# zfwangDP/X2-GNN

Hardware: AMD Instinct MI355X
Metric: molecules/sec (fwd+bwd) on QM9 U0, batch=128, 1/2/4/8 MI355X (higher is better)
Workload: dtype fp32; 1 GPU; xgnn_poly U0 train step (config.json: L=4, D=128, H=16, sbf 7x6), S160, fwd+loss+bwd+allreduce+clip+Adam+EMA; per_gpu_batch=128, global_batch=128, line_nodes_per_gpu=21058, triplets_per_gpu=194060, parallelism=dp1, hip_graph=True

## Files before the change

### x2-gnn_amd/csrc/attention_center.hip

```cpp
#include <math.h>

#include <type_traits>

#include "common.hpp"
#include "../../include/x2g_staged.h"

namespace x2g {
namespace {

constexpr int kCD = 128;
constexpr float kCEps = 1e-16f;
typedef float cf4 __attribute__((ext_vector_type(4)));

__device__ __forceinline__ cf4 ld4(const float* p) { return *reinterpret_cast<const cf4*>(p); }
__device__ __forceinline__ void st4(float* p, cf4 v) { *reinterpret_cast<cf4*>(p) = v; }

template <int LPH>
__device__ __forceinline__ float head_sum(float v) {
  return group_sum<LPH>(v);
}

template <int LPH>
__device__ __forceinline__ float qk_logit(cf4 qv, cf4 kr, float sqrt_c) {
  float dot = __fmul_rn(qv[0], kr[0]);
  dot = __fmaf_rn(qv[1], kr[1], dot);
  dot = __fmaf_rn(qv[2], kr[2], dot);
  dot = __fmaf_rn(qv[3], kr[3], dot);
  return __fdiv_rn(head_sum<LPH>(dot), sqrt_c);
}

__device__ __forceinline__ float half_sum(float v, int half) {
  v = half32_sum_hi(v);
  const float lo = lane_bcast(v, 31), hi = lane_bcast(v, 63);
  return half ? hi : lo;
}

constexpr int kFactBatch = 4;
constexpr int kSfL = 7;
constexpr int kSfR = 6;
constexpr int kSfK = kSfL * kSfR;

constexpr int kMaxMembers = 32;

struct UnitRows {
  int* LN;
  int* RI;
  int* ER;
  int* MA;
  int* MI;
  int* NRS;
};

__host__ __device__ constexpr size_t unit_rows_lds(int rows) {
  return ((static_cast<size_t>(3) * rows + 2 * kMaxMembers + 4) * 4 + 15) / 16 * 16;
}

__device__ __forceinline__ UnitRows unit_rows_carve(int* p, int max_rows) {
  UnitRows u;
  u.NRS = p;
  u.MA = p + 4;
  u.MI = u.MA + kMaxMembers;
  u.LN = u.MI + kMaxMembers;
  u.RI = u.LN + max_rows;
  u.ER = u.RI + max_rows;
  return u;
}

__device__ __forceinline__ void unit_rows_build(const UnitRows& u, const int32_t* __restrict__ order,
                                                const int32_t* __restrict__ packs, int64_t unit,
                                                const int32_t* __restrict__ rowptr,
                                                const int32_t* __restrict__ src_row,
                                                const int4* __restrict__ info, int max_rows) {
  if (threadIdx.x >= 64) return;
  const int lane = threadIdx.x;
  int64_t m0 = unit, m1 = unit + 1;
  if (packs) {
    m0 = packs[unit];
    m1 = packs[unit + 1];
  }
  const int M = static_cast<int>(m1 - m0);
  int b = 0, r0 = 0, n = 0, er = 0;
  if (info) {
    if (lane < M) {
      const int4 v = info[m0 + lane];
      b = v.x;
      r0 = v.y;
      n = v.z;
      er = src_row ? v.w : 0;
    }
  } else {
    if (lane < M) {
      b = order ? order[m0 + lane] : static_cast<int>(m0 + lane);
      r0 = rowptr[b];
      n = rowptr[b + 1] - r0;
    }
    er = (src_row && n > 0) ? src_row[r0] : 0;
  }
  int inc = n;
#pragma unroll
  for (int o = 1; o < 64; o <<= 1) {
    const int v = __shfl_up(inc, o);
    if (lane >= o) inc += v;
  }
  const int base = inc - n;
  const int total = __shfl(inc, 63);
  if (total > max_rows) {
    if (lane == 63) {
      u.NRS[0] = 0;
      u.NRS[1] = 0;
    }
    return;
  }
  if (lane < M) {
    u.MA[lane] = b;
    u.MI[lane] = base | n << 16;
    for (int r = 0; r < n; ++r) {
      u.LN[base + r] = r0 + r;
      u.RI[base + r] = base | n << 16;
      u.ER[base + r] = er;
    }
  }
  if (lane == 63) {
    u.NRS[0] = inc;
    u.NRS[1] = M;
  }
}

struct FwdCenterArgs {
  const float *q, *k, *v, *skip, *edge;
  const int32_t* src_row;
  const float* sp;
  int64_t t_base;
  const int32_t *atom_rowptr, *edge_rev, *rev_trip;
  const int32_t* order;
  int64_t atom0, n_atoms;
  int H;
  float sqrt_c;
  float *out, *alpha, *smax, *sden;
  float2* row_stats;
};

template <int LPH, int WAVES, int B, bool EDGE>
__global__ void __launch_bounds__(64 * WAVES) attn_fwd_center_kernel(const FwdCenterArgs a) {
  extern __shared__ cf4 lds[];
  const int64_t b = a.order ? static_cast<int64_t>(a.order[a.atom0 + blockIdx.x]) : a.atom0 + blockIdx.x;
  const int r0 = uniform(a.atom_rowptr[b]);
  const int n = uniform(a.atom_rowptr[b + 1]) - r0;
  if (n <= 0) return;
  cf4* ke = lds;
  cf4* ve = lds + n * 32;
  const int tid = threadIdx.x;
  const int l32 = tid & 31, half = (tid >> 5) & 1, wave = tid >> 6;
  const int owner = 2 * wave + half;
  const int head = l32 / LPH;
  const bool leader = (l32 % LPH) == 0;
  const int c0 = 4 * l32;
  int i = owner;
  int d = 0, tb = 0;
// ... 424 lines not shown
          if constexpr (PREFETCH) load(j0 + B, yn, tn);
          cf4 sv[B];
          float lg[B];
          float mb = -INFINITY;
#pragma unroll
          for (int uu = 0; uu < B; ++uu) {
            const int j = j0 + uu;
            const bool ok = j < n && j != i;
            const int jr = (j < t1 ? j : t1 - 1) - t0;
            float yl[kSfL];
            yl[0] = dpp_mov<0x150>(yv[uu]);
            yl[1] = dpp_mov<0x151>(yv[uu]);
            yl[2] = dpp_mov<0x152>(yv[uu]);
            yl[3] = dpp_mov<0x153>(yv[uu]);
            yl[4] = dpp_mov<0x154>(yv[uu]);
            yl[5] = dpp_mov<0x155>(yv[uu]);
            yl[6] = dpp_mov<0x156>(yv[uu]);
            cf4 s4 = bias4;
            if constexpr (DROP && RMAX > 2 && B > 2) s4 = ld4(a.bias + c0);
#pragma unroll
            for (int l = 0; l < kSfL; ++l) s4 += yl[l] * P[(jr * kSfL + l) * 32 + l32];
            sv[uu] = s4;
            if constexpr (STORE) {
              if (a.sp && ok) st4(a.sp + static_cast<int64_t>(tt[uu]) * kCD + c0, s4);
            }
            const cf4 kr = KE[jr * 32 + l32];
            const float logit = qk_logit<LPH>(qv, kr, a.sqrt_c);
            lg[uu] = ok ? logit : -INFINITY;
            mb = fmaxf(mb, lg[uu]);
            if constexpr (STORE) {
              if (a.alpha && ok && leader) a.alpha[static_cast<int64_t>(tt[uu]) * a.H + head] = logit;
            }
          }
          const float m_new = fmaxf(m[r], mb);
          const float corr = m_new == -INFINITY ? 1.f : expf(m[r] - m_new);
          den[r] *= corr;
          acc[r] *= corr;
#pragma unroll
          for (int uu = 0; uu < B; ++uu) {
            const int j = j0 + uu;
            const float p = lg[uu] == -INFINITY ? 0.f : expf(lg[uu] - m_new);
            const cf4 vr = VE[((j < t1 ? j : t1 - 1) - t0) * 32 + l32];
            den[r] += p;
            if constexpr (DROP)
              acc[r] += (p * (drop_keep(dkey, tt[uu], head, a.H) ? dkey.scale : 0.f)) * (vr * sv[uu]);
            else
              acc[r] += p * (vr * sv[uu]);
          }
          m[r] = m_new;
          if constexpr (PREFETCH) {
#pragma unroll
            for (int uu = 0; uu < B; ++uu) {
              yv[uu] = yn[uu];
              tt[uu] = tn[uu];
            }
          } else {
            load(j0 + B, yv, tt);
          }
        }
      }
    }
  }
#pragma unroll
  for (int r = 0; r < RMAX; ++r) {
    if (owner + NO * r >= n) continue;
    const int dd = DDs[owner + NO * r];
    const int64_t drow = static_cast<int64_t>(dd) * kCD + c0;
    const float inv = 1.0f / (den[r] + kCEps);
    const cf4 o = acc[r] * inv + ld4(a.skip + drow);
    st4(a.out + drow, o);
    if (a.row_stats) {
      const float mu = half_sum(o[0] + o[1] + o[2] + o[3], half) / static_cast<float>(kCD);
      const cf4 dv = o - mu;
      const float q2 = half_sum(dv[0] * dv[0] + dv[1] * dv[1] + dv[2] * dv[2] + dv[3] * dv[3], half);
      if (l32 == 0) a.row_stats[dd] = make_float2(mu, q2);
    }
    if (leader) {
      a.smax[static_cast<int64_t>(dd) * a.H + head] = m[r];
      a.sden[static_cast<int64_t>(dd) * a.H + head] = den[r];
    }
  }
}

constexpr size_t fwd_sf_tiled_lds() {
  return static_cast<size_t>(kTileRows) * ((2 + kSfL) * kCD + kSfK) * 4 + 2 * X2G_CENTER_MAX_DEGREE * 4;
}

template <int LPH, bool DROP>
int fwd_sf_tiled_launch(const FwdSfArgs& a, bool edge, int max_degree, hipStream_t st) {
  constexpr int W = 8, B = 4;
  const size_t lds = fwd_sf_tiled_lds();
  const unsigned grid = static_cast<unsigned>(a.n_atoms);
  auto go = [&](auto kern) -> int {
    const hipError_t e = hipFuncSetAttribute(reinterpret_cast<const void*>(kern),
                                             hipFuncAttributeMaxDynamicSharedMemorySize, static_cast<int>(lds));
    if (e != hipSuccess) return static_cast<int>(e);
    kern<<<grid, 64 * W, lds, st>>>(a);
    return last_launch_status();
  };
  constexpr int NO = 2 * W;
  const bool store = a.alpha || a.sp || a.pp;
  auto pick = [&](auto rmax) -> int {
    constexpr int R = decltype(rmax)::value;
    if constexpr (DROP) {
      static_assert(R <= 4, "no RMAX 8 dropout instance");
      constexpr int BN = LPH == 1 && R > 2 ? 2 : B;
      return edge ? go(attn_fwd_center_sf_tiled_kernel<LPH, W, B, true, R, true, true>)
                  : go(attn_fwd_center_sf_tiled_kernel<LPH, W, BN, false, R, true, true>);
    } else {
      if (store)
        return edge ? go(attn_fwd_center_sf_tiled_kernel<LPH, W, B, true, R, true, false>)
                    : go(attn_fwd_center_sf_tiled_kernel<LPH, W, B, false, R, true, false>);
      return edge ? go(attn_fwd_center_sf_tiled_kernel<LPH, W, B, true, R, false, false>)
                  : go(attn_fwd_center_sf_tiled_kernel<LPH, W, B, false, R, false, false>);
    }
  };
  if (max_degree <= 2 * NO) return pick(std::integral_constant<int, 2>{});
  if (max_degree <= 4 * NO) return pick(std::integral_constant<int, 4>{});
  if constexpr (DROP)
    return X2G_EUNSUPPORTED;
  else
    return pick(std::integral_constant<int, 8>{});
}

template <int LPH>
int fwd_center_launch(const FwdCenterArgs& a, bool edge, int max_degree, hipStream_t st) {
  constexpr int W = 4, B = 8;
  const size_t lds = static_cast<size_t>(2) * max_degree * kCD * sizeof(float);
  const unsigned grid = static_cast<unsigned>(a.n_atoms);
  auto go = [&](auto kern) -> int {
    if (lds > 64 * 1024) {
      const hipError_t e = hipFuncSetAttribute(reinterpret_cast<const void*>(kern),
                                               hipFuncAttributeMaxDynamicSharedMemorySize, static_cast<int>(lds));
      if (e != hipSuccess) return static_cast<int>(e);
    }
    kern<<<grid, 64 * W, lds, st>>>(a);
    return last_launch_status();
  };
  return edge ? go(attn_fwd_center_kernel<LPH, W, B, true>) : go(attn_fwd_center_kernel<LPH, W, B, false>);
}

struct BwdCenterArgs {
  const float *q, *k, *v, *edge;
  const int32_t* src_row;
  const float *sp, *alpha, *smax, *sden, *dout, *y;
  const float *pp, *bias;
  const int32_t *atom_rowptr, *edge_rev, *rev_trip;
  const int32_t* order;
  int64_t n_atoms, T;
  int H;
  float inv_sqrt_c;
  float sqrt_c;
  float *dq, *dk, *dv, *gfold, *d_edge, *gw;
  const int64_t* drop_key;
  uint32_t drop_salt, drop_thr;
  float drop_scale;
};

template <int H>
__host__ __device__ constexpr size_t bwd_center_lds(int n) {
  return static_cast<size_t>(n) * 4 * kCD * 4
         + static_cast<size_t>(n) * H * 4 * 3
         + static_cast<size_t>(n) * 4 * 2;
}

template <int LPH, int WAVES, int B, bool EDGE, bool FACT, bool DROP>
__global__ void __launch_bounds__(64 * WAVES, 4) attn_bwd_center_kernel(const BwdCenterArgs a) {
  static_assert(FACT || !DROP, "the dropout instances are the P-row ones");
  constexpr int H = 32 / LPH;
  extern __shared__ cf4 lds[];
  const int64_t b = a.order ? static_cast<int64_t>(a.order[blockIdx.x]) : static_cast<int64_t>(blockIdx.x);
  const int r0 = uniform(a.atom_rowptr[b]);
  const int n = uniform(a.atom_rowptr[b + 1]) - r0;
  const int tid = threadIdx.x;
  const int l32 = tid & 31, half = (tid >> 5) & 1, wave = tid >> 6;
  const int owner = 2 * wave + half;
  constexpr int NO = 2 * WAVES;
  const int head = l32 / LPH;
  const bool leader = (l32 % LPH) == 0;
  const int c0 = 4 * l32;
  DropKey dkey{};
  if constexpr (DROP) dkey = drop_key(a.drop_key, a.drop_salt, a.drop_thr, a.drop_scale);
  if (n <= 0) {
    if (a.d_edge && tid < 32) st4(a.d_edge + b * kCD + c0, cf4{0.f, 0.f, 0.f, 0.f});
    return;
  }
  cf4* KE = lds;
  cf4* GO = KE + n * 32;
  cf4* QI = GO + n * 32;
  cf4* DE = QI + n * 32;
  float* MX = reinterpret_cast<float*>(DE + n * 32);
  float* IV = MX + n * H;
  float* RHO = IV + n * H;
  int* TB = reinterpret_cast<int*>(RHO + n * H);
  int* DI = TB + n;
  const int64_t e_row = EDGE ? static_cast<int64_t>(uniform(a.src_row[r0])) * kCD : 0;
  for (int idx = tid; idx < n; idx += 64 * WAVES) {
    TB[idx] = a.rev_trip[r0 + idx];
    DI[idx] = a.edge_rev[r0 + idx];
  }
  __syncthreads();
  constexpr int NT = 64 * WAVES;
  if (n * 32 <= 2 * NT && n * H <= NT) {
    cf4 kk[2], gg[2], qq[2];
    const int c = tid & 31;
    const cf4 e4 = EDGE ? ld4(a.edge + e_row + 4 * c) : cf4{0.f, 0.f, 0.f, 0.f};
#pragma unroll
    for (int u = 0; u < 2; ++u) {
      int j = (tid + u * NT) >> 5;
      j = j < n ? j : n - 1;
      const int64_t d = DI[j];
      kk[u] = ld4(a.k + static_cast<int64_t>(r0 + j) * kCD + 4 * c);
      gg[u] = ld4(a.dout + d * kCD + 4 * c);
      qq[u] = ld4(a.q + d * kCD + 4 * c);
    }
    const int sidx = tid < n * H ? tid : 0;
    const int si = sidx / H, sh = sidx - si * H;
    const int64_t sd = DI[si];
    const float mx = a.smax[sd * H + sh], dn = a.sden[sd * H + sh];
#pragma unroll
    for (int u = 0; u < 2; ++u) {
      const int idx = tid + u * NT;
      if (idx < n * 32) {
        KE[idx] = kk[u] + e4;
        GO[idx] = gg[u];
        QI[idx] = qq[u];
      }
    }
    if (tid < n * H) {
      MX[tid] = mx;
      IV[tid] = 1.0f / (dn + kCEps);
    }
  } else {
    for (int idx = tid; idx < n * 32; idx += NT) {
      const int j = idx >> 5, c = idx & 31;
      const int64_t d = DI[j];
      const cf4 e4 = EDGE ? ld4(a.edge + e_row + 4 * c) : cf4{0.f, 0.f, 0.f, 0.f};
      KE[idx] = ld4(a.k + static_cast<int64_t>(r0 + j) * kCD + 4 * c) + e4;
      GO[idx] = ld4(a.dout + d * kCD + 4 * c);
      QI[idx] = ld4(a.q + d * kCD + 4 * c);
    }
    for (int idx = tid; idx < n * H; idx += NT) {
      const int i = idx / H, h = idx - i * H;
      const int64_t d = DI[i];
      MX[idx] = a.smax[d * H + h];
      IV[idx] = 1.0f / (a.sden[d * H + h] + kCEps);
    }
  }
  __syncthreads();
  const int nt = n - 1;
  auto rsrc = [](const void* p, int64_t bytes) {
    return __builtin_amdgcn_make_buffer_rsrc(const_cast<void*>(p), static_cast<short>(0),
                                             static_cast<int>(bytes < 0x7fffffff ? bytes : 0x7fffffff), 0x00020000);
  };
  const __amdgpu_buffer_rsrc_t sp_r = rsrc(a.sp, a.T * kCD * 4);
  const __amdgpu_buffer_rsrc_t al_r = rsrc(a.alpha, a.T * H * 4);
  const __amdgpu_buffer_rsrc_t y_r = rsrc(a.y, a.T * 8 * 4);
  const __amdgpu_buffer_rsrc_t ag_r = rsrc(a.gw, a.T * H * 8);
  auto ldf = [](__amdgpu_buffer_rsrc_t r, int off) {
    return __builtin_bit_cast(float, __builtin_amdgcn_raw_buffer_load_b32(r, off, 0, 0));
  };
  auto ldag = [&](int t) {
    return __builtin_bit_cast(float2, __builtin_amdgcn_raw_buffer_load_b64(ag_r, (t * H + head) * 8, 0, 0));
  };
  auto trip = [&](int i, int j) {
    int pos = j - (j > i ? 1 : 0);
    pos = pos < nt ? pos : nt - 1;
    return TB[i] + pos;
  };
  for (int j = owner; j < n; j += NO) {
    const int64_t srow = static_cast<int64_t>(r0 + j) * kCD + c0;
    cf4 ue = ld4(a.v + srow);
    if (EDGE) ue += ld4(a.edge + e_row + c0);
    cf4 dv = {0.f, 0.f, 0.f, 0.f};
    cf4 pj[FACT ? kSfL : 1], bias4 = {0.f, 0.f, 0.f, 0.f};
    if constexpr (FACT) {
#pragma unroll
      for (int l = 0; l < kSfL; ++l) pj[l] = ld4(a.pp + (static_cast<int64_t>(r0 + j) * kSfL + l) * kCD + c0);
      bias4 = ld4(a.bias + c0);
    }
    auto batch = [&](int i0, auto bb) {
      constexpr int BB = decltype(bb)::value;
      cf4 sv[FACT ? 1 : BB];
      float yv[FACT ? BB : 1];
      float al[BB];
      int tt[BB];
#pragma unroll
      for (int u = 0; u < BB; ++u) {
        const int i = i0 + u < n ? i0 + u : n - 1;
        tt[u] = trip(i, j);
        if constexpr (FACT)
          yv[u] = ldf(y_r, (tt[u] * 8 + (l32 & 7)) * 4);
        else
          sv[u] = __builtin_bit_cast(cf4, __builtin_amdgcn_raw_buffer_load_b128(sp_r, tt[u] * (kCD * 4) + c0 * 4, 0, 0));
        al[u] = ldf(al_r, (tt[u] * H + head) * 4);
      }
#pragma unroll
      for (int u = 0; u < BB; ++u) {
        const int i = i0 + u < n ? i0 + u : n - 1;
        const bool ok = i0 + u < n && i != j;
        cf4 st;
        if constexpr (FACT) {
          float yl[kSfL];
          yl[0] = dpp_mov<0x150>(yv[u]);
          yl[1] = dpp_mov<0x151>(yv[u]);
          yl[2] = dpp_mov<0x152>(yv[u]);
          yl[3] = dpp_mov<0x153>(yv[u]);
          yl[4] = dpp_mov<0x154>(yv[u]);
          yl[5] = dpp_mov<0x155>(yv[u]);
          yl[6] = dpp_mov<0x156>(yv[u]);
          st = bias4;
#pragma unroll
          for (int l = 0; l < kSfL; ++l) st += yl[l] * pj[l];
        } else {
          st = sv[u];
        }
        const float at = ok ? expf(al[u] - MX[i * H + head]) * IV[i * H + head] : 0.f;
        const cf4 go = GO[i * 32 + l32];
        const cf4 gu = go * ue;
        float gp = gu[0] * st[0];
        gp = fmaf(gu[1], st[1], gp);
        gp = fmaf(gu[2], st[2], gp);
        gp = fmaf(gu[3], st[3], gp);
        const float g = head_sum<LPH>(gp);
        if (ok && leader) *reinterpret_cast<float2*>(a.gw + (static_cast<int64_t>(tt[u]) * H + head) * 2) = make_float2(g, at);
        dv += at * (go * st);
      }
    };
    if constexpr (FACT) {
      constexpr int BB = kFactBatch;
      if (nt > 0) {
        const cf4 kj = KE[j * 32 + l32];
        float yv[BB];
        int tt[BB];
        auto load = [&](int i0, float (&y_)[BB], int (&t_)[BB]) {
#pragma unroll
          for (int u = 0; u < BB; ++u) {
            const int i = i0 + u < n ? i0 + u : n - 1;
            t_[u] = trip(i, j);
            y_[u] = ldf(y_r, (t_[u] * 8 + (l32 & 7)) * 4);
          }
        };
        load(0, yv, tt);
        for (int i0 = 0; i0 < n; i0 += BB) {
          float yn[BB];
          int tn[BB];
          load(i0 + BB, yn, tn);
#pragma unroll
          for (int u = 0; u < BB; ++u) {
            const int i = i0 + u < n ? i0 + u : n - 1;
            const bool ok = i0 + u < n && i != j;
            float yl[kSfL];
            yl[0] = dpp_mov<0x150>(yv[u]);
            yl[1] = dpp_mov<0x151>(yv[u]);
            yl[2] = dpp_mov<0x152>(yv[u]);
            yl[3] = dpp_mov<0x153>(yv[u]);
            yl[4] = dpp_mov<0x154>(yv[u]);
            yl[5] = dpp_mov<0x155>(yv[u]);
            yl[6] = dpp_mov<0x156>(yv[u]);
            cf4 st = bias4;
#pragma unroll
            for (int l = 0; l < kSfL; ++l) st += yl[l] * pj[l];
            const float logit = qk_logit<LPH>(QI[i * 32 + l32], kj, a.sqrt_c);
            const float at = ok ? expf(logit - MX[i * H + head]) * IV[i * H + head] : 0.f;
            const cf4 go = GO[i * 32 + l32];
            const cf4 gu = go * ue;
            float gp = gu[0] * st[0];
            gp = fmaf(gu[1], st[1], gp);
            gp = fmaf(gu[2], st[2], gp);
            gp = fmaf(gu[3], st[3], gp);
            const float g = head_sum<LPH>(gp);
            if constexpr (DROP) {
              const float rk = drop_keep(dkey, tt[u], head, H) ? dkey.scale : 0.f;
              __builtin_amdgcn_raw_buffer_store_b64(__builtin_bit_cast(__attribute__((ext_vector_type(2))) unsigned,
                                                                       make_float2(g * rk, rk != 0.f ? at : -at)),
                                                    ag_r, (ok && leader) ? (tt[u] * H + head) * 8 : static_cast<int>(0x80000000u),
                                                    0, 0);
              dv += (at * rk) * (go * st);
            } else {
              __builtin_amdgcn_raw_buffer_store_b64(__builtin_bit_cast(__attribute__((ext_vector_type(2))) unsigned,
                                                                       make_float2(g, at)),
                                                    ag_r, (ok && leader) ? (tt[u] * H + head) * 8 : static_cast<int>(0x80000000u),
                                                    0, 0);
              dv += at * (go * st);
            }
          }
#pragma unroll
          for (int u = 0; u < BB; ++u) {
            yv[u] = yn[u];
            tt[u] = tn[u];
          }
        }
      }
    } else if (nt > 0) {
      int i0 = 0;
      for (; n - i0 > B / 2; i0 += B) batch(i0, std::integral_constant<int, B>{});
      if (i0 < n) batch(i0, std::integral_constant<int, B / 2>{});
    }
    st4(a.dv + srow, dv);
    DE[j * 32 + l32] = dv;
  }
  __threadfence_block();
  __syncthreads();
  for (int i = owner; i < n; i += NO) {
    float rho = 0.f;
    for (int p0 = 0; p0 < nt; p0 += 8) {
      float at[8], g[8];
#pragma unroll
      for (int u = 0; u < 8; ++u) {
        const float2 ag = ldag(TB[i] + (p0 + u < nt ? p0 + u : nt - 1));
        g[u] = ag.x;
        at[u] = ag.y;
      }
#pragma unroll
      for (int u = 0; u < 8; ++u)
        if (p0 + u < nt) {
          if constexpr (DROP)
            rho = fmaf(fabsf(at[u]), g[u], rho);
          else
            rho = fmaf(at[u], g[u], rho);
        }
    }
    if (leader) RHO[i * H + head] = rho;
  }
  __syncthreads();
  for (int o = owner; o < n; o += NO) {
    const int64_t srow = static_cast<int64_t>(r0 + o) * kCD + c0;
    cf4 ue = ld4(a.v + srow);
    if (EDGE) ue += ld4(a.edge + e_row + c0);
    cf4 dk = {0.f, 0.f, 0.f, 0.f}, dq = {0.f, 0.f, 0.f, 0.f};
    cf4 G[8];
#pragma unroll
    for (int l = 0; l < 8; ++l) G[l] = cf4{0.f, 0.f, 0.f, 0.f};
    const float rho_o = RHO[o * H + head];
    auto batch = [&](int x0, auto bb) {
      constexpr int BB = decltype(bb)::value;
      float ats[BB], gs[BB], yv[BB], atd[BB], gd[BB];
#pragma unroll
      for (int u = 0; u < BB; ++u) {
        const int x = x0 + u < n ? x0 + u : n - 1;
        const int ts = trip(x, o), td = trip(o, x);
        const float2 ags = ldag(ts), agd = ldag(td);
        gs[u] = ags.x;
        ats[u] = ags.y;
        yv[u] = ldf(y_r, (ts * 8 + (l32 & 7)) * 4);
        gd[u] = agd.x;
        atd[u] = agd.y;
      }
#pragma unroll
      for (int u = 0; u < BB; ++u) {
        const int x = x0 + u < n ? x0 + u : n - 1;
        const bool ok = x0 + u < n && x != o;
        const float as = ok ? (DROP ? fabsf(ats[u]) : ats[u]) : 0.f, ad = ok ? (DROP ? fabsf(atd[u]) : atd[u]) : 0.f;
        const float ws = as * (gs[u] - RHO[x * H + head]) * a.inv_sqrt_c;
        dk += ws * QI[x * 32 + l32];
        const float wd = ad * (gd[u] - rho_o) * a.inv_sqrt_c;
        dq += wd * KE[x * 32 + l32];
        cf4 ds;
        if constexpr (DROP)
          ds = (GO[x * 32 + l32] * ue) * (as * (__float_as_int(ats[u]) < 0 ? 0.f : dkey.scale));
        else
          ds = (GO[x * 32 + l32] * ue) * as;
        float yl[8];
        yl[0] = dpp_mov<0x150>(yv[u]);
        yl[1] = dpp_mov<0x151>(yv[u]);
        yl[2] = dpp_mov<0x152>(yv[u]);
        yl[3] = dpp_mov<0x153>(yv[u]);
        yl[4] = dpp_mov<0x154>(yv[u]);
        yl[5] = dpp_mov<0x155>(yv[u]);
        yl[6] = dpp_mov<0x156>(yv[u]);
        yl[7] = dpp_mov<0x157>(yv[u]);
#pragma unroll
        for (int l = 0; l < 8; ++l) G[l] += ds * yl[l];
      }
    };
    if (nt > 0) {
      int x0 = 0;
      for (; n - x0 > B / 2; x0 += B) batch(x0, std::integral_constant<int, B>{});
      if (x0 < n) batch(x0, std::integral_constant<int, B / 2>{});
    }
    st4(a.dk + srow, dk);
    st4(a.dq + static_cast<int64_t>(DI[o]) * kCD + c0, dq);
    float* gf = a.gfold + static_cast<int64_t>(r0 + o) * 8 * kCD + c0;
#pragma unroll
    for (int l = 0; l < 8; ++l) st4(gf + l * kCD, G[l]);
    DE[o * 32 + l32] += dk;
  }
  if (a.d_edge) {
    __syncthreads();
    if (tid < 32) {
      cf4 s = DE[l32];
      for (int j = 1; j < n; ++j) s += DE[j * 32 + l32];
      st4(a.d_edge + b * kCD + c0, s);
    }
  }
}

template <int LPH, bool DROP>
int bwd_center_launch(const BwdCenterArgs& a, bool edge, int max_degree, hipStream_t st) {
  constexpr int W = 4, B = 8;
  constexpr int H = 32 / LPH;
  const size_t lds = bwd_center_lds<H>(max_degree);
  if (lds > 160 * 1024) return X2G_EUNSUPPORTED;
  const unsigned grid = static_cast<unsigned>(a.n_atoms);
  auto go = [&](auto kern) -> int {
    if (lds > 64 * 1024) {
      const hipError_t e = hipFuncSetAttribute(reinterpret_cast<const void*>(kern),
                                               hipFuncAttributeMaxDynamicSharedMemorySize, static_cast<int>(lds));
      if (e != hipSuccess) return static_cast<int>(e);
    }
    kern<<<grid, 64 * W, lds, st>>>(a);
    return last_launch_status();
  };
  if (a.pp)
    return edge ? go(attn_bwd_center_kernel<LPH, W, B, true, true, DROP>)
                : go(attn_bwd_center_kernel<LPH, W, B, false, true, DROP>);
  if constexpr (!DROP)
    return edge ? go(attn_bwd_center_kernel<LPH, W, B, true, false, false>)
                : go(attn_bwd_center_kernel<LPH, W, B, false, false, false>);
  return X2G_EUNSUPPORTED;
}

struct DropIn {
  float p;
  const int64_t* key;
  uint32_t salt;
};

template <class Args>
int drop_args(const DropIn* drop, Args* a) {
  if (!drop) return X2G_OK;
  if (!drop->key || !drop_params(drop->p, &a->drop_thr, &a->drop_scale)) return X2G_EINVAL;
  a->drop_key = drop->key;
  a->drop_salt = drop->salt;
  return X2G_OK;
}

}
}

using namespace x2g;

X2G_API size_t x2g_sbf_attention_bwd_center_lds(int32_t max_degree, int32_t heads) {
  if (max_degree < 0 || heads <= 0) return 0;
  const int n = max_degree > 0 ? max_degree : 1;
  return static_cast<size_t>(n) * 4 * kCD * 4 + static_cast<size_t>(n) * heads * 12 + static_cast<size_t>(n) * 8;
}

static int bwd_center_entry(const float* q, const float* k, const float* v, const float* edge,
                                         const int32_t* src_row, int edge_mode, const float* sbfproj,
                                         const float* sbf_p, const float* b_sbf,
                                         const float* sph_y, const int32_t* atom_rowptr, const int32_t* edge_rev,
                                         const int32_t* rev_trip, const int32_t* atom_order, const float* alpha_raw,
                                         const float* seg_max,
                                         const float* seg_den, const float* dout, int64_t num_atoms,
                                         int32_t max_degree, int64_t num_edges, int64_t num_triplets, int32_t heads,
                                         int32_t channels, float* dq, float* dk, float* dv, float* radial_grad,
                                         float* d_edge_atom, float* g_work, void* stream, const DropIn* drop) {
  if (num_atoms < 0 || num_edges < 0 || num_triplets < 0 || heads <= 0 || channels <= 0) return X2G_EINVAL;
  if (edge_mode != X2G_EDGE_NONE && edge_mode != X2G_EDGE_PER_DST) return X2G_EUNSUPPORTED;
  if (heads * channels != kCD || channels % 4 || max_degree < 0 || max_degree > X2G_CENTER_MAX_DEGREE)
    return X2G_EUNSUPPORTED;
  if (x2g_sbf_attention_bwd_center_lds(max_degree, heads) > 160 * 1024) return X2G_EUNSUPPORTED;
  if (num_triplets * (sbf_p ? int64_t(heads) * 8 : int64_t(kCD) * 4) >= (int64_t(1) << 31)) return X2G_EUNSUPPORTED;
  BwdCenterArgs a{};
  if (const int rc = drop_args(drop, &a)) return rc;
  if (num_atoms == 0) return X2G_OK;
  if (!sbfproj == !sbf_p || (sbf_p && !b_sbf)) return X2G_EINVAL;
  if (drop && !sbf_p) return X2G_EUNSUPPORTED;
  if (num_edges > 0 && (!q || !k || !v || !sph_y || !atom_rowptr || !edge_rev || !rev_trip ||
                        (!alpha_raw && !sbf_p) || !seg_max || !seg_den || !dout || !dq || !dk || !dv ||
                        !radial_grad || (num_triplets > 0 && !g_work)))
    return X2G_EINVAL;
  if (!atom_rowptr) return X2G_EINVAL;
  if (edge_mode == X2G_EDGE_PER_DST && (!edge || !src_row)) return X2G_EINVAL;
  const auto al = [](const void* p, int m) { return p == nullptr || reinterpret_cast<uintptr_t>(p) % m == 0; };
  if (!al(q, 16) || !al(k, 16) || !al(v, 16) || !al(edge, 16) || !al(sbfproj, 16) || !al(dout, 16) || !al(dq, 16) ||
      !al(dk, 16) || !al(dv, 16) || !al(radial_grad, 16) || !al(d_edge_atom, 16) || !al(sbf_p, 16) || !al(b_sbf, 16))
    return X2G_EUNSUPPORTED;
  a.pp = sbf_p; a.bias = b_sbf;
  a.q = q; a.k = k; a.v = v; a.edge = edge; a.src_row = src_row; a.sp = sbfproj; a.alpha = alpha_raw;
  a.smax = seg_max; a.sden = seg_den; a.dout = dout; a.y = sph_y; a.atom_rowptr = atom_rowptr; a.edge_rev = edge_rev;
  a.rev_trip = rev_trip; a.order = atom_order; a.n_atoms = num_atoms; a.T = num_triplets; a.H = heads;
  a.inv_sqrt_c = static_cast<float>(1.0 / sqrt(static_cast<double>(channels)));
  a.sqrt_c = static_cast<float>(sqrt(static_cast<double>(channels)));
  a.dq = dq; a.dk = dk; a.dv = dv; a.gfold = radial_grad; a.d_edge = d_edge_atom; a.gw = g_work;
  const int md = max_degree > 0 ? max_degree : 1;
  const bool edge_on = edge_mode == X2G_EDGE_PER_DST;
  hipStream_t st = as_stream(stream);
  switch (channels / 4) {
    case 1: return drop ? bwd_center_launch<1, true>(a, edge_on, md, st) : bwd_center_launch<1, false>(a, edge_on, md, st);
    case 2: return drop ? bwd_center_launch<2, true>(a, edge_on, md, st) : bwd_center_launch<2, false>(a, edge_on, md, st);
    case 4: return drop ? bwd_center_launch<4, true>(a, edge_on, md, st) : bwd_center_launch<4, false>(a, edge_on, md, st);
    case 8: return drop ? bwd_center_launch<8, true>(a, edge_on, md, st) : bwd_center_launch<8, false>(a, edge_on, md, st);
    default: return X2G_EUNSUPPORTED;
  }
}

X2G_API int x2g_sbf_attention_bwd_center(const float* q, const float* k, const float* v, const float* edge,
                                         const int32_t* src_row, int edge_mode, const float* sbfproj,
                                         const float* sbf_p, const float* b_sbf,
                                         const float* sph_y, const int32_t* atom_rowptr, const int32_t* edge_rev,
                                         const int32_t* rev_trip, const int32_t* atom_order, const float* alpha_raw,
                                         const float* seg_max,
                                         const float* seg_den, const float* dout, int64_t num_atoms,
                                         int32_t max_degree, int64_t num_edges, int64_t num_triplets, int32_t heads,
                                         int32_t channels, float* dq, float* dk, float* dv, float* radial_grad,
                                         float* d_edge_atom, float* g_work, void* stream) {
  return bwd_center_entry(q, k, v, edge, src_row, edge_mode, sbfproj, sbf_p, b_sbf, sph_y, atom_rowptr, edge_rev,
                          rev_trip, atom_order, alpha_raw, seg_max, seg_den, dout, num_atoms, max_degree, num_edges,
                          num_triplets, heads, channels, dq, dk, dv, radial_grad, d_edge_atom, g_work, stream,
                          nullptr);
}

X2G_API int x2g_sbf_attention_bwd_center_drop(const float* q, const float* k, const float* v, const float* edge,
                                              const int32_t* src_row, int edge_mode, const float* sbfproj,
                                              const float* sbf_p, const float* b_sbf, const float* sph_y,
                                              const int32_t* atom_rowptr, const int32_t* edge_rev,
                                              const int32_t* rev_trip, const int32_t* atom_order,
                                              const float* alpha_raw, const float* seg_max, const float* seg_den,
                                              const float* dout, int64_t num_atoms, int32_t max_degree,
                                              int64_t num_edges, int64_t num_triplets, int32_t heads,
                                              int32_t channels, float* dq, float* dk, float* dv, float* radial_grad,
                                              float* d_edge_atom, float* g_work, void* stream, float drop_p,
                                              const int64_t* drop_key, uint32_t salt) {
  const DropIn drop{drop_p, drop_key, salt};
  return bwd_center_entry(q, k, v, edge, src_row, edge_mode, sbfproj, sbf_p, b_sbf, sph_y, atom_rowptr, edge_rev,
                          rev_trip, atom_order, alpha_raw, seg_max, seg_den, dout, num_atoms, max_degree, num_edges,
                          num_triplets, heads, channels, dq, dk, dv, radial_grad, d_edge_atom, g_work, stream, &drop);
}

X2G_API int x2g_sbf_attention_fwd_center(const float* q, const float* k, const float* v, const float* skip,
                                         const float* edge, const int32_t* src_row, int edge_mode,
                                         const float* sbfproj, int64_t t_base, const int32_t* atom_rowptr,
                                         const int32_t* edge_rev, const int32_t* rev_trip, const int32_t* atom_order,
                                         int64_t atom0,
                                         int64_t n_atoms, int32_t max_degree, int64_t num_edges,
                                         int64_t num_triplets, int32_t heads, int32_t channels, float* out,
                                         float* alpha_raw, float* seg_max, float* seg_den, float* row_stats,
                                         void* stream) {
  if (n_atoms < 0 || atom0 < 0 || num_edges < 0 || num_triplets < 0 || heads <= 0 || channels <= 0)
    return X2G_EINVAL;
  if (edge_mode != X2G_EDGE_NONE && edge_mode != X2G_EDGE_PER_DST) return X2G_EUNSUPPORTED;
  if (heads * channels != kCD || channels % 4 || max_degree < 0 || max_degree > X2G_CENTER_MAX_DEGREE)
    return X2G_EUNSUPPORTED;
  if (n_atoms == 0 || num_edges == 0) return X2G_OK;
  if (!q || !k || !v || !skip || !sbfproj || !atom_rowptr || !edge_rev || !rev_trip || !out || !seg_max || !seg_den)
    return X2G_EINVAL;
  if (edge_mode == X2G_EDGE_PER_DST && (!edge || !src_row)) return X2G_EINVAL;
  const auto al = [](const void* p, int m) { return p == nullptr || reinterpret_cast<uintptr_t>(p) % m == 0; };
  if (!al(q, 16) || !al(k, 16) || !al(v, 16) || !al(skip, 16) || !al(edge, 16) || !al(sbfproj, 16) || !al(out, 16) ||
      !al(row_stats, 8))
    return X2G_EUNSUPPORTED;
  FwdCenterArgs a{};
  a.q = q; a.k = k; a.v = v; a.skip = skip; a.edge = edge; a.src_row = src_row; a.sp = sbfproj; a.t_base = t_base;
  a.atom_rowptr = atom_rowptr; a.edge_rev = edge_rev; a.rev_trip = rev_trip; a.order = atom_order; a.atom0 = atom0;
  a.n_atoms = n_atoms; a.H = heads; a.sqrt_c = static_cast<float>(sqrt(static_cast<double>(channels)));
  a.out = out; a.alpha = alpha_raw; a.smax = seg_max; a.sden = seg_den;
  a.row_stats = reinterpret_cast<float2*>(row_stats);
  const int md = max_degree > 0 ? max_degree : 1;
  const bool edge_on = edge_mode == X2G_EDGE_PER_DST;
  hipStream_t st = as_stream(stream);
  switch (channels / 4) {
    case 1: return fwd_center_launch<1>(a, edge_on, md, st);
    case 2: return fwd_center_launch<2>(a, edge_on, md, st);
    case 4: return fwd_center_launch<4>(a, edge_on, md, st);
    case 8: return fwd_center_launch<8>(a, edge_on, md, st);
    default: return X2G_EUNSUPPORTED;
  }
}

static int fwd_center_sf_entry(const float* q, const float* k, const float* v, const float* skip,
                                            const float* edge, const int32_t* src_row, int edge_mode,
                                            const float* radial, const float* sph_y, const float* w_sbf,
                                            const float* b_sbf, const int32_t* atom_rowptr, const int32_t* edge_rev,
                                            const int32_t* rev_trip, const int32_t* atom_order,
                                            const int32_t* pack_ptr, const int32_t* atom_info, int64_t unit0,
                                            int64_t n_units,
                                            int32_t max_rows, int64_t num_edges, int64_t num_triplets, int32_t heads,
                                            int32_t channels, float* out, float* alpha_raw, float* seg_max,
                                            float* seg_den, float* row_stats, float* sbfproj_out, float* sbf_p_out,
                                            void* stream, const DropIn* drop) {
  if (n_units < 0 || unit0 < 0 || num_edges < 0 || num_triplets < 0 || heads <= 0 || channels <= 0)
    return X2G_EINVAL;
  if (edge_mode != X2G_EDGE_NONE && edge_mode != X2G_EDGE_PER_DST) return X2G_EUNSUPPORTED;
  if (heads * channels != kCD || channels % 4 || max_rows < 0 || max_rows > X2G_CENTER_MAX_DEGREE ||
      fwd_sf_lds(max_rows > 0 ? max_rows : 1) > 160 * 1024)
    return X2G_EUNSUPPORTED;
  FwdSfArgs a{};
  if (const int rc = drop_args(drop, &a)) return rc;
  if (n_units == 0 || num_edges == 0) return X2G_OK;
  if (!q || !k || !v || !skip || !radial || !sph_y || !w_sbf || !b_sbf || !atom_rowptr || !edge_rev || !rev_trip ||
      !out || !seg_max || !seg_den || (pack_ptr && !atom_order))
    return X2G_EINVAL;
  if (edge_mode == X2G_EDGE_PER_DST && (!edge || !src_row)) return X2G_EINVAL;
  const auto al = [](const void* p, int m) { return p == nullptr || reinterpret_cast<uintptr_t>(p) % m == 0; };
  if (!al(q, 16) || !al(k, 16) || !al(v, 16) || !al(skip, 16) || !al(edge, 16) || !al(out, 16) || !al(b_sbf, 16) ||
      !al(sbfproj_out, 16) || !al(sbf_p_out, 16) || !al(row_stats, 8) || !al(atom_info, 16))
    return X2G_EUNSUPPORTED;
  a.info = reinterpret_cast<const int4*>(atom_info);
  a.pp = sbf_p_out;
  a.q = q; a.k = k; a.v = v; a.skip = skip; a.edge = edge; a.src_row = src_row; a.radial = radial; a.y = sph_y;
  a.w = w_sbf; a.bias = b_sbf; a.atom_rowptr = atom_rowptr; a.edge_rev = edge_rev; a.rev_trip = rev_trip;
  a.order = atom_order; a.packs = pack_ptr; a.atom0 = unit0; a.n_atoms = n_units;
  a.max_rows = max_rows > 0 ? max_rows : 1; a.H = heads;
  a.sqrt_c = static_cast<float>(sqrt(static_cast<double>(channels)));
  a.out = out; a.alpha = alpha_raw; a.smax = seg_max; a.sden = seg_den; a.sp = sbfproj_out;
  a.row_stats = reinterpret_cast<float2*>(row_stats);
  const bool edge_on = edge_mode == X2G_EDGE_PER_DST;
  hipStream_t st = as_stream(stream);
  switch (channels / 4) {
    case 1: return drop ? fwd_sf_launch<1, true>(a, edge_on, st) : fwd_sf_launch<1, false>(a, edge_on, st);
    case 2: return drop ? fwd_sf_launch<2, true>(a, edge_on, st) : fwd_sf_launch<2, false>(a, edge_on, st);
    case 4: return drop ? fwd_sf_launch<4, true>(a, edge_on, st) : fwd_sf_launch<4, false>(a, edge_on, st);
    case 8: return drop ? fwd_sf_launch<8, true>(a, edge_on, st) : fwd_sf_launch<8, false>(a, edge_on, st);
    default: return X2G_EUNSUPPORTED;
  }
}

X2G_API int x2g_sbf_attention_fwd_center_sf(const float* q, const float* k, const float* v, const float* skip,
                                            const float* edge, const int32_t* src_row, int edge_mode,
                                            const float* radial, const float* sph_y, const float* w_sbf,
                                            const float* b_sbf, const int32_t* atom_rowptr, const int32_t* edge_rev,
                                            const int32_t* rev_trip, const int32_t* atom_order,
                                            const int32_t* pack_ptr, const int32_t* atom_info, int64_t unit0,
                                            int64_t n_units,
                                            int32_t max_rows, int64_t num_edges, int64_t num_triplets, int32_t heads,
                                            int32_t channels, float* out, float* alpha_raw, float* seg_max,
                                            float* seg_den, float* row_stats, float* sbfproj_out, float* sbf_p_out,
                                            void* stream) {
  return fwd_center_sf_entry(q, k, v, skip, edge, src_row, edge_mode, radial, sph_y, w_sbf, b_sbf, atom_rowptr,
                             edge_rev, rev_trip, atom_order, pack_ptr, atom_info, unit0, n_units, max_rows, num_edges,
                             num_triplets, heads, channels, out, alpha_raw, seg_max, seg_den, row_stats, sbfproj_out,
                             sbf_p_out, stream, nullptr);
}

X2G_API int x2g_sbf_attention_fwd_center_sf_drop(const float* q, const float* k, const float* v, const float* skip,
                                                 const float* edge, const int32_t* src_row, int edge_mode,
                                                 const float* radial, const float* sph_y, const float* w_sbf,
                                                 const float* b_sbf, const int32_t* atom_rowptr,
                                                 const int32_t* edge_rev, const int32_t* rev_trip,
                                                 const int32_t* atom_order, const int32_t* pack_ptr,
                                                 const int32_t* atom_info, int64_t unit0, int64_t n_units,
                                                 int32_t max_rows, int64_t num_edges, int64_t num_triplets,
                                                 int32_t heads, int32_t channels, float* out, float* alpha_raw,
                                                 float* seg_max, float* seg_den, float* row_stats,
                                                 float* sbfproj_out, float* sbf_p_out, void* stream, float drop_p,
                                                 const int64_t* drop_key, uint32_t salt) {
  const DropIn drop{drop_p, drop_key, salt};
  return fwd_center_sf_entry(q, k, v, skip, edge, src_row, edge_mode, radial, sph_y, w_sbf, b_sbf, atom_rowptr,
                             edge_rev, rev_trip, atom_order, pack_ptr, atom_info, unit0, n_units, max_rows, num_edges,
                             num_triplets, heads, channels, out, alpha_raw, seg_max, seg_den, row_stats, sbfproj_out,
                             sbf_p_out, stream, &drop);
}

X2G_API size_t x2g_sbf_attention_fwd_center_sf_tiled_lds(void) { return fwd_sf_tiled_lds(); }

static int fwd_center_sf_tiled_entry(const float* q, const float* k, const float* v, const float* skip,
                                                  const float* edge, const int32_t* src_row, int edge_mode,
                                                  const float* radial, const float* sph_y, const float* w_sbf,
                                                  const float* b_sbf, const int32_t* atom_rowptr,
                                                  const int32_t* edge_rev, const int32_t* rev_trip,
                                                  const int32_t* atom_order, const int32_t* pack_ptr,
                                                  const int32_t* atom_info, int64_t unit0, int64_t n_units,
                                                  int32_t max_degree, int32_t skip_rows, int64_t num_edges,
                                                  int64_t num_triplets,
                                                  int32_t heads, int32_t channels, float* out, float* alpha_raw,
                                                  float* seg_max, float* seg_den, float* row_stats,
                                                  float* sbfproj_out, float* sbf_p_out, void* stream,
                                                  const DropIn* drop) {
  if (n_units < 0 || unit0 < 0 || num_edges < 0 || num_triplets < 0 || heads <= 0 || channels <= 0)
    return X2G_EINVAL;
  if (edge_mode != X2G_EDGE_NONE && edge_mode != X2G_EDGE_PER_DST) return X2G_EUNSUPPORTED;
  if (heads * channels != kCD || channels % 4 || max_degree < 0 || max_degree > X2G_CENTER_MAX_DEGREE)
    return X2G_EUNSUPPORTED;
  if (drop && max_degree > 64) return X2G_EUNSUPPORTED;
  FwdSfArgs a{};
  if (const int rc = drop_args(drop, &a)) return rc;
  if (n_units == 0 || num_edges == 0) return X2G_OK;
  if (!q || !k || !v || !skip || !radial || !sph_y || !w_sbf || !b_sbf || !atom_rowptr || !edge_rev || !rev_trip ||
      !out || !seg_max || !seg_den || (pack_ptr && !atom_order))
    return X2G_EINVAL;
// ... 89 lines not shown
```

### x2-gnn_amd/x2gnn/_lib.py

```python
from __future__ import annotations

import ctypes
import keyword
import os
import re

import torch

_HERE = os.path.dirname(os.path.abspath(__file__))
LIB_PATH = os.environ.get("X2G_LIB", os.path.join(os.path.dirname(_HERE), "lib", "libx2g.so"))
HEADER_PATH = os.environ.get("X2G_HEADER",
                             os.path.join(os.path.dirname(os.path.dirname(_HERE)), "include", "x2g.h"))
STAGED_HEADER_PATH = os.path.join(os.path.dirname(HEADER_PATH), "x2g_staged.h")
MULTI_HEADER_PATH = os.path.join(os.path.dirname(HEADER_PATH), "x2g_multi.h")

_SCALARS = {"int64_t": ctypes.c_int64, "int32_t": ctypes.c_int32, "uint32_t": ctypes.c_uint32, "int": ctypes.c_int,
            "float": ctypes.c_float, "double": ctypes.c_double, "size_t": ctypes.c_size_t}


class _Consts(dict):

    def __init__(self):
        super().__init__()
        self.other = {}

    def __missing__(self, name):
        if name in self.other:
            raise ValueError(f"#define {name} is not an integer literal: {self.other[name]!r}")
        raise KeyError(name)


def _ctype(spec, decl, known, ret=False):
    words = [w for w in re.findall(r"\w+|\*", spec) if w != "const"]
    base, stars = words[:1], words[1:]
    if len(base) == 1 and all(s == "*" for s in stars):
        if not stars and base[0] in _SCALARS:
            return _SCALARS[base[0]]
        if stars and (base[0] in _SCALARS or base[0] in known or base[0] in ("void", "char")):
            return ctypes.c_char_p if ret and base[0] == "char" and len(stars) == 1 else ctypes.c_void_p
    raise ValueError(f"x2g.h: unknown type {spec.strip()!r} in: {decl}")


def _split(item, decl):
    m = re.fullmatch(r"([\w\s*]+?)\s*\b(\w+)", item.strip())
    if not m:
        raise ValueError(f"x2g.h: cannot read {item.strip()!r} in: {decl}")
    return m[1], m[2]


def parse_header(text):
    text = re.sub(r"/\*.*?\*/|//[^\n]*", " ", text, flags=re.S)
    text = re.sub(r"^[ \t]*#[ \t]*ifdef[ \t]+__cplusplus\b.*?^[ \t]*#[ \t]*endif\b[^\n]*", "", text, flags=re.S | re.M)
    consts = _Consts()
    for name, value in re.findall(r"^[ \t]*#[ \t]*define[ \t]+(\w+)(.*)$", text, flags=re.M):
        name = name[4:] if name.startswith("X2G_") else name
        try:
            consts[name] = int(value.strip(), 0)
        except ValueError:
            consts.other[name] = value.strip()
    text = re.sub(r"^[ \t]*#.*$", "", text, flags=re.M)

    structs = {}

    def struct(m):
        decl = " ".join(m[0].split())
        fields = []
        for item in filter(str.strip, m[1].split(";")):
            spec, name = _split(item, decl)
            fields.append((name + "_" if keyword.iskeyword(name) else name, _ctype(spec, decl, structs)))
        structs[m[2]] = type(m[2], (ctypes.Structure,), {"_fields_": fields, "__doc__": f"{m[2]} (include/x2g.h)."})
        return ""

    text = re.sub(r"\btypedef\s+struct\s*\{([^{}]*)\}\s*(\w+)\s*;", struct, text)

    signatures, restypes = {}, {}
    for decl in filter(None, (" ".join(d.split()) for d in text.split(";"))):
        m = re.fullmatch(r"([\w\s*]+?)\s*\b(\w+)\s*\(([^()]*)\)", decl)
        if not m:
            raise ValueError(f"x2g.h: cannot read the declaration: {decl}")
        args = [] if m[3].strip() == "void" else m[3].split(",")
        signatures[m[2]] = [_ctype(_split(a, decl)[0], decl, structs) for a in args]
        restypes[m[2]] = _ctype(m[1], decl, structs, ret=True)
    return signatures, restypes, structs, consts


def _read_header():
    if not os.path.exists(HEADER_PATH):
        raise RuntimeError(f"x2g.h not found at {HEADER_PATH}: set X2G_HEADER to the header libx2g.so was built from")
    with open(HEADER_PATH) as f:
        return f.read()


def _read_functions(path):
    if not os.path.exists(path):
        return {}, {}
    with open(path) as f:
        sig, res, structs, consts = parse_header(f.read())
    if structs or consts:
        raise ValueError(f"{os.path.basename(path)} declares more than functions: "
                         f"{sorted(structs) + sorted(consts)}")
    return sig, res


SIGNATURES, RESTYPES, STRUCTS, CONSTS = parse_header(_read_header())
STAGED_SIGNATURES, STAGED_RESTYPES = _read_functions(STAGED_HEADER_PATH)
MULTI_SIGNATURES, MULTI_RESTYPES = _read_functions(MULTI_HEADER_PATH)

_lib = None


def load():
    global _lib
    if _lib is None:
        if not os.path.exists(LIB_PATH):
            raise RuntimeError(f"libx2g.so not found at {LIB_PATH}: build it (make -C x2-gnn_amd) first")
        lib = ctypes.CDLL(LIB_PATH)
        for name, args in SIGNATURES.items():
            fn = getattr(lib, name)
            fn.argtypes = args
            fn.restype = RESTYPES[name]
        for sigs, res in ((STAGED_SIGNATURES, STAGED_RESTYPES), (MULTI_SIGNATURES, MULTI_RESTYPES)):
            for name, args in sigs.items():
                fn = getattr(lib, name, None)
                if fn is not None:
                    fn.argtypes = args
                    fn.restype = res[name]
        _lib = lib
    return _lib


def ptr(t):
    if t is None:
        return None
    return ctypes.c_void_p(t.data_ptr())


def stream_ptr(device=None):
    return ctypes.c_void_p(torch.cuda.current_stream(device).cuda_stream)


def check(rc: int, name: str):
    if rc != 0:
        msg = load().x2g_status_string(rc).decode()
        raise RuntimeError(f"{name} failed with status {rc}: {msg}")


def call(name: str, *args):
    check(getattr(load(), name)(*args), name)
```

Measured before the change: 59570 molecules/s.

## Keep per-pair attention gradient scratch in LDS for low-degree atoms in center backward

Adds an LDS-resident scratch path to the center attention backward kernel. For atoms whose degree fits a computed cap, the per-triplet (g, alpha) pairs are stored in and read from shared memory instead of the global g_work buffer. The goal is to remove global round trips between the two backward phases. The LDS allocation per block grows to the larger of the two layouts, which can reduce occupancy, and the dual path adds a branch and more code size. Higher-degree atoms, dropout runs and non-factored runs keep the existing global path.

```diff
diff --git a/include/x2g_staged_cap.h b/include/x2g_staged_cap.h
--- /dev/null
+++ b/include/x2g_staged_cap.h
@@ -0,0 +1,25 @@
+#ifndef X2G_STAGED_CAP_H
+#define X2G_STAGED_CAP_H
+
+#include "x2g.h"
+
+#ifdef __cplusplus
+extern "C" {
+#endif
+
+int x2g_sbf_attention_bwd_center_cap(const float* q, const float* k, const float* v, const float* edge,
+                                     const int32_t* src_row, int edge_mode, const float* sbfproj,
+                                     const float* sbf_p, const float* b_sbf, const float* sph_y,
+                                     const int32_t* atom_rowptr, const int32_t* edge_rev, const int32_t* rev_trip,
+                                     const int32_t* atom_order, const float* alpha_raw, const float* seg_max,
+                                     const float* seg_den, const float* dout, int64_t num_atoms,
+                                     int32_t max_degree, int64_t num_edges, int64_t num_triplets, int32_t heads,
+                                     int32_t channels, float* dq, float* dk, float* dv, float* radial_grad,
+                                     float* d_edge_atom, float* g_work, void* stream,
+                                     int32_t lds_scratch_max_degree);
+
+#ifdef __cplusplus
+}
+#endif
+
+#endif
diff --git a/x2-gnn_amd/csrc/attention_center.hip b/x2-gnn_amd/csrc/attention_center.hip
--- a/x2-gnn_amd/csrc/attention_center.hip
+++ b/x2-gnn_amd/csrc/attention_center.hip
@@ -4,6 +4,7 @@
 
 #include "common.hpp"
 #include "../../include/x2g_staged.h"
+#include "../../include/x2g_staged_cap.h"
 
 namespace x2g {
 namespace {
@@ -734,6 +735,7 @@
   float inv_sqrt_c;
   float sqrt_c;
   float *dq, *dk, *dv, *gfold, *d_edge, *gw;
+  int lds_cap;
   const int64_t* drop_key;
   uint32_t drop_salt, drop_thr;
   float drop_scale;
@@ -746,14 +748,18 @@
          + static_cast<size_t>(n) * 4 * 2;
 }
 
-template <int LPH, int WAVES, int B, bool EDGE, bool FACT, bool DROP>
-__global__ void __launch_bounds__(64 * WAVES, 4) attn_bwd_center_kernel(const BwdCenterArgs a) {
+template <int H>
+__host__ __device__ constexpr size_t bwd_center_lds_pairs(int n) {
+  return (static_cast<size_t>(n) * (n - 1) + 1) * H * 8;
+}
+
+template <int LPH, int WAVES, int B, bool EDGE, bool FACT, bool DROP, bool LSCR>
+__device__ __forceinline__ void attn_bwd_center_body(const BwdCenterArgs& a, const int64_t b, const int r0,
+                                                     const int n) {
   static_assert(FACT || !DROP, "the dropout instances are the P-row ones");
+  static_assert(!LSCR || (FACT && !DROP), "the LDS-scratch instances are the plain P-row ones");
   constexpr int H = 32 / LPH;
   extern __shared__ cf4 lds[];
-  const int64_t b = a.order ? static_cast<int64_t>(a.order[blockIdx.x]) : static_cast<int64_t>(blockIdx.x);
-  const int r0 = uniform(a.atom_rowptr[b]);
-  const int n = uniform(a.atom_rowptr[b + 1]) - r0;
   const int tid = threadIdx.x;
   const int l32 = tid & 31, half = (tid >> 5) & 1, wave = tid >> 6;
   const int owner = 2 * wave + half;
@@ -776,6 +782,7 @@
   float* RHO = IV + n * H;
   int* TB = reinterpret_cast<int*>(RHO + n * H);
   int* DI = TB + n;
+  float2* LSC = reinterpret_cast<float2*>(DI + n);
   const int64_t e_row = EDGE ? static_cast<int64_t>(uniform(a.src_row[r0])) * kCD : 0;
   for (int idx = tid; idx < n; idx += 64 * WAVES) {
     TB[idx] = a.rev_trip[r0 + idx];
@@ -843,12 +850,21 @@
     return __builtin_bit_cast(float, __builtin_amdgcn_raw_buffer_load_b32(r, off, 0, 0));
   };
   auto ldag = [&](int t) {
-    return __builtin_bit_cast(float2, __builtin_amdgcn_raw_buffer_load_b64(ag_r, (t * H + head) * 8, 0, 0));
+    if constexpr (LSCR)
+      return LSC[t * H + head];
+    else
+      return __builtin_bit_cast(float2, __builtin_amdgcn_raw_buffer_load_b64(ag_r, (t * H + head) * 8, 0, 0));
   };
   auto trip = [&](int i, int j) {
     int pos = j - (j > i ? 1 : 0);
     pos = pos < nt ? pos : nt - 1;
     return TB[i] + pos;
+  };
+  auto sblock = [&](int i) { return LSCR ? i * nt : TB[i]; };
+  auto strip = [&](int i, int j) {
+    int pos = j - (j > i ? 1 : 0);
+    pos = pos < nt ? pos : nt - 1;
+    return sblock(i) + pos;
   };
   for (int j = owner; j < n; j += NO) {
     const int64_t srow = static_cast<int64_t>(r0 + j) * kCD + c0;
@@ -959,6 +975,9 @@
                                                     ag_r, (ok && leader) ? (tt[u] * H + head) * 8 : static_cast<int>(0x80000000u),
                                                     0, 0);
               dv += (at * rk) * (go * st);
+            } else if constexpr (LSCR) {
+              LSC[((ok && leader) ? strip(i, j) : n * nt) * H + head] = make_float2(g, at);
+              dv += at * (go * st);
             } else {
               __builtin_amdgcn_raw_buffer_store_b64(__builtin_bit_cast(__attribute__((ext_vector_type(2))) unsigned,
                                                                        make_float2(g, at)),
@@ -990,7 +1009,7 @@
       float at[8], g[8];
 #pragma unroll
       for (int u = 0; u < 8; ++u) {
-        const float2 ag = ldag(TB[i] + (p0 + u < nt ? p0 + u : nt - 1));
+        const float2 ag = ldag(sblock(i) + (p0 + u < nt ? p0 + u : nt - 1));
         g[u] = ag.x;
         at[u] = ag.y;
       }
@@ -1022,7 +1041,7 @@
       for (int u = 0; u < BB; ++u) {
         const int x = x0 + u < n ? x0 + u : n - 1;
         const int ts = trip(x, o), td = trip(o, x);
-        const float2 ags = ldag(ts), agd = ldag(td);
+        const float2 ags = ldag(LSCR ? strip(x, o) : ts), agd = ldag(LSCR ? strip(o, x) : td);
         gs[u] = ags.x;
         ats[u] = ags.y;
         yv[u] = ldf(y_r, (ts * 8 + (l32 & 7)) * 4);
@@ -1078,12 +1097,39 @@
   }
 }
 
+template <int LPH, int WAVES, int B, bool EDGE, bool FACT, bool DROP, bool DUAL = false>
+__global__ void __launch_bounds__(64 * WAVES, 4) attn_bwd_center_kernel(const BwdCenterArgs a) {
+  const int64_t b = a.order ? static_cast<int64_t>(a.order[blockIdx.x]) : static_cast<int64_t>(blockIdx.x);
+  const int r0 = uniform(a.atom_rowptr[b]);
+  const int n = uniform(a.atom_rowptr[b + 1]) - r0;
+  if (!DUAL || n > a.lds_cap)
+    attn_bwd_center_body<LPH, WAVES, B, EDGE, FACT, DROP, false>(a, b, r0, n);
+  else
+    attn_bwd_center_body<LPH, WAVES, B, EDGE, FACT, DROP, DUAL>(a, b, r0, n);
+}
+
+template <int H>
+constexpr int bwd_center_lds_cap() {
+  int c = 1;
+  while (bwd_center_lds<H>(c + 1) + bwd_center_lds_pairs<H>(c + 1) <= 160 * 1024 / 4) ++c;
+  return c;
+}
+
 template <int LPH, bool DROP>
-int bwd_center_launch(const BwdCenterArgs& a, bool edge, int max_degree, hipStream_t st) {
+int bwd_center_launch(const BwdCenterArgs& a0, bool edge, int max_degree, int cap, hipStream_t st) {
   constexpr int W = 4, B = 8;
   constexpr int H = 32 / LPH;
-  const size_t lds = bwd_center_lds<H>(max_degree);
+  size_t lds = bwd_center_lds<H>(max_degree);
   if (lds > 160 * 1024) return X2G_EUNSUPPORTED;
+  if (cap < 0) cap = bwd_center_lds_cap<H>();
+  if (DROP || !a0.pp) cap = 0;
+  BwdCenterArgs a = a0;
+  a.lds_cap = cap < max_degree ? cap : max_degree;
+  if (cap > 0) {
+    const size_t lds_c = bwd_center_lds<H>(a.lds_cap) + bwd_center_lds_pairs<H>(a.lds_cap);
+    if (lds_c > 160 * 1024) return X2G_EUNSUPPORTED;
+    lds = lds_c > lds ? lds_c : lds;
+  }
   const unsigned grid = static_cast<unsigned>(a.n_atoms);
   auto go = [&](auto kern) -> int {
     if (lds > 64 * 1024) {
@@ -1094,6 +1140,11 @@
     kern<<<grid, 64 * W, lds, st>>>(a);
     return last_launch_status();
   };
+  if constexpr (!DROP) {
+    if (cap > 0)
+      return edge ? go(attn_bwd_center_kernel<LPH, W, B, true, true, false, true>)
+                  : go(attn_bwd_center_kernel<LPH, W, B, false, true, false, true>);
+  }
   if (a.pp)
     return edge ? go(attn_bwd_center_kernel<LPH, W, B, true, true, DROP>)
                 : go(attn_bwd_center_kernel<LPH, W, B, false, true, DROP>);
@@ -1138,7 +1189,9 @@
                                          const float* seg_den, const float* dout, int64_t num_atoms,
                                          int32_t max_degree, int64_t num_edges, int64_t num_triplets, int32_t heads,
                                          int32_t channels, float* dq, float* dk, float* dv, float* radial_grad,
-                                         float* d_edge_atom, float* g_work, void* stream, const DropIn* drop) {
+                                         float* d_edge_atom, float* g_work, void* stream, const DropIn* drop,
+                                         int cap) {
+  if (cap < -1) return X2G_EINVAL;
   if (num_atoms < 0 || num_edges < 0 || num_triplets < 0 || heads <= 0 || channels <= 0) return X2G_EINVAL;
   if (edge_mode != X2G_EDGE_NONE && edge_mode != X2G_EDGE_PER_DST) return X2G_EUNSUPPORTED;
   if (heads * channels != kCD || channels % 4 || max_degree < 0 || max_degree > X2G_CENTER_MAX_DEGREE)
@@ -1171,10 +1224,10 @@
   const bool edge_on = edge_mode == X2G_EDGE_PER_DST;
   hipStream_t st = as_stream(stream);
   switch (channels / 4) {
-    case 1: return drop ? bwd_center_launch<1, true>(a, edge_on, md, st) : bwd_center_launch<1, false>(a, edge_on, md, st);
-    case 2: return drop ? bwd_center_launch<2, true>(a, edge_on, md, st) : bwd_center_launch<2, false>(a, edge_on, md, st);
-    case 4: return drop ? bwd_center_launch<4, true>(a, edge_on, md, st) : bwd_center_launch<4, false>(a, edge_on, md, st);
-    case 8: return drop ? bwd_center_launch<8, true>(a, edge_on, md, st) : bwd_center_launch<8, false>(a, edge_on, md, st);
+    case 1: return drop ? bwd_center_launch<1, true>(a, edge_on, md, 0, st) : bwd_center_launch<1, false>(a, edge_on, md, cap, st);
+    case 2: return drop ? bwd_center_launch<2, true>(a, edge_on, md, 0, st) : bwd_center_launch<2, false>(a, edge_on, md, cap, st);
+    case 4: return drop ? bwd_center_launch<4, true>(a, edge_on, md, 0, st) : bwd_center_launch<4, false>(a, edge_on, md, cap, st);
+    case 8: return drop ? bwd_center_launch<8, true>(a, edge_on, md, 0, st) : bwd_center_launch<8, false>(a, edge_on, md, cap, st);
     default: return X2G_EUNSUPPORTED;
   }
 }
@@ -1192,7 +1245,24 @@
   return bwd_center_entry(q, k, v, edge, src_row, edge_mode, sbfproj, sbf_p, b_sbf, sph_y, atom_rowptr, edge_rev,
                           rev_trip, atom_order, alpha_raw, seg_max, seg_den, dout, num_atoms, max_degree, num_edges,
                           num_triplets, heads, channels, dq, dk, dv, radial_grad, d_edge_atom, g_work, stream,
-                          nullptr);
+                          nullptr, -1);
+}
+
+X2G_API int x2g_sbf_attention_bwd_center_cap(const float* q, const float* k, const float* v, const float* edge,
+                                             const int32_t* src_row, int edge_mode, const float* sbfproj,
+                                             const float* sbf_p, const float* b_sbf, const float* sph_y,
+                                             const int32_t* atom_rowptr, const int32_t* edge_rev,
+                                             const int32_t* rev_trip, const int32_t* atom_order,
+                                             const float* alpha_raw, const float* seg_max, const float* seg_den,
+                                             const float* dout, int64_t num_atoms, int32_t max_degree,
+                                             int64_t num_edges, int64_t num_triplets, int32_t heads,
+                                             int32_t channels, float* dq, float* dk, float* dv, float* radial_grad,
+                                             float* d_edge_atom, float* g_work, void* stream,
+                                             int32_t lds_scratch_max_degree) {
+  return bwd_center_entry(q, k, v, edge, src_row, edge_mode, sbfproj, sbf_p, b_sbf, sph_y, atom_rowptr, edge_rev,
+                          rev_trip, atom_order, alpha_raw, seg_max, seg_den, dout, num_atoms, max_degree, num_edges,
+                          num_triplets, heads, channels, dq, dk, dv, radial_grad, d_edge_atom, g_work, stream,
+                          nullptr, lds_scratch_max_degree);
 }
 
 X2G_API int x2g_sbf_attention_bwd_center_drop(const float* q, const float* k, const float* v, const float* edge,
@@ -1209,7 +1279,7 @@
   const DropIn drop{drop_p, drop_key, salt};
   return bwd_center_entry(q, k, v, edge, src_row, edge_mode, sbfproj, sbf_p, b_sbf, sph_y, atom_rowptr, edge_rev,
                           rev_trip, atom_order, alpha_raw, seg_max, seg_den, dout, num_atoms, max_degree, num_edges,
-                          num_triplets, heads, channels, dq, dk, dv, radial_grad, d_edge_atom, g_work, stream, &drop);
+                          num_triplets, heads, channels, dq, dk, dv, radial_grad, d_edge_atom, g_work, stream, &drop, 0);
 }
 
 X2G_API int x2g_sbf_attention_fwd_center(const float* q, const float* k, const float* v, const float* skip,
diff --git a/x2-gnn_amd/x2gnn/_lib.py b/x2-gnn_amd/x2gnn/_lib.py
--- a/x2-gnn_amd/x2gnn/_lib.py
+++ b/x2-gnn_amd/x2gnn/_lib.py
@@ -13,6 +13,7 @@
                              os.path.join(os.path.dirname(os.path.dirname(_HERE)), "include", "x2g.h"))
 STAGED_HEADER_PATH = os.path.join(os.path.dirname(HEADER_PATH), "x2g_staged.h")
 MULTI_HEADER_PATH = os.path.join(os.path.dirname(HEADER_PATH), "x2g_multi.h")
+CAP_HEADER_PATH = os.path.join(os.path.dirname(HEADER_PATH), "x2g_staged_cap.h")
 
 _SCALARS = {"int64_t": ctypes.c_int64, "int32_t": ctypes.c_int32, "uint32_t": ctypes.c_uint32, "int": ctypes.c_int,
             "float": ctypes.c_float, "double": ctypes.c_double, "size_t": ctypes.c_size_t}
@@ -105,6 +106,7 @@
 SIGNATURES, RESTYPES, STRUCTS, CONSTS = parse_header(_read_header())
 STAGED_SIGNATURES, STAGED_RESTYPES = _read_functions(STAGED_HEADER_PATH)
 MULTI_SIGNATURES, MULTI_RESTYPES = _read_functions(MULTI_HEADER_PATH)
+CAP_SIGNATURES, CAP_RESTYPES = _read_functions(CAP_HEADER_PATH)
 
 _lib = None
 
@@ -119,7 +121,8 @@
             fn = getattr(lib, name)
             fn.argtypes = args
             fn.restype = RESTYPES[name]
-        for sigs, res in ((STAGED_SIGNATURES, STAGED_RESTYPES), (MULTI_SIGNATURES, MULTI_RESTYPES)):
+        for sigs, res in ((STAGED_SIGNATURES, STAGED_RESTYPES), (MULTI_SIGNATURES, MULTI_RESTYPES),
+                          (CAP_SIGNATURES, CAP_RESTYPES)):
             for name, args in sigs.items():
                 fn = getattr(lib, name, None)
                 if fn is not None:
```

After: 59960 molecules/s (median of 6 runs). About the same (+0.6%).
